# nullmax-vision/SimPB

Measured on AMD Instinct MI355X. Metric: frames/sec (6-cam sample) + MSDeformAttn HBM GB/s, R50 704x256 @1/2/4/8 GPU, higher is better.
Workload: dtype f32

## Files before the change

### include/simpb_hip.h

```cpp
#ifndef SIMPB_HIP_H
#define SIMPB_HIP_H

#ifdef __cplusplus
extern "C" {
#endif

#define SIMPB_OK 0
#define SIMPB_EINVAL 1
#define SIMPB_ELAUNCH 2

#define SIMPB_RECORD3D_WIDTH 15

int simpb_abi_version(void);

const char* simpb_last_error(void);

#define SIMPB_KERNEL_DAF 1
#define SIMPB_KERNEL_MSDA 2
int simpb_timing_enable(int capacity);
int simpb_timing_read(int kernel_id, float* ms_out, int max_n);
void simpb_timing_reset(void);

int simpb_deformable_aggregation_forward(
    float* output, const float* mc_ms_feat, const int* spatial_shape, const int* scale_start_index,
// ... 91 lines not shown
#define SIMPB_SURFACE_RGBA 13
int simpb_preprocess_planes_nhwc4_f16(void* out, const void* src, const void* image_table, void* mid, const int* kx,
                                      const int* xlo, const int* xn, const int* ky, const int* ylo, const int* yn,
                                      const void* lut, int num_images, int src_height, int src_width, int out_height,
                                      int out_width, int taps_x, int taps_y, int src_row0, int src_rows, int flip, int swap_rb,
                                      int format, long long pitch, long long chroma_pitch, long long chroma_offset,
                                      long long chroma2_offset, long long image_stride, int yoff, int iy, int irv, int igu,
                                      int igv, int ibu, void* stream);

int simpb_preprocess_mid_pitch(int out_width);

#define SIMPB_RIG_MAX_CAMS 16
typedef struct simpb_rig_camera {
  int format, src_height, src_width;
  int src_row0, src_rows, taps_x, taps_y, flip;
  long long pitch, chroma_pitch, chroma_offset;
  int kx_offset, x_offset, ky_offset, y_offset, mid_row;
  int yoff, iy, irv, igu, igv, ibu;
  long long chroma2_offset;
} simpb_rig_camera;
int simpb_preprocess_rig_nhwc4_f16(void* out, const void* image_table, void* mid, const int* kx, const int* xlo, const int* xn,
                                   const int* ky, const int* ylo, const int* yn, const void* lut, const simpb_rig_camera* cams,
                                   int num_cams, int num_images, int out_height, int out_width, int kx_len, int x_len, int ky_len,
                                   int y_len, int mid_rows, int swap_rb, void* stream);

#define SIMPB_PREPROCESS_MAX_ROLL_SIZE 8192
int simpb_preprocess_roll_nhwc4_f16(void* out, const void* src, const void* image_table, void* mid, const int* kx,
                                    const int* xlo, const int* xn, const int* ky, const int* ylo, const int* yn, const void* lut,
                                    int num_images, int src_height, int src_width, int out_height, int out_width, int taps_x,
                                    int taps_y, int src_row0, int src_rows, int flip, int swap_rb, int format, long long pitch,
                                    long long chroma_pitch, long long chroma_offset, long long chroma2_offset,
                                    long long image_stride, int yoff, int iy, int irv, int igu, int igv, int ibu, const int* roll,
                                    int roll_cams, void* stream);
int simpb_preprocess_rig_roll_nhwc4_f16(void* out, const void* image_table, void* mid, const int* kx, const int* xlo,
                                        const int* xn, const int* ky, const int* ylo, const int* yn, const void* lut,
                                        const simpb_rig_camera* cams, int num_cams, int num_images, int out_height, int out_width,
                                        int kx_len, int x_len, int ky_len, int y_len, int mid_rows, int swap_rb, const int* roll,
                                        void* stream);

#define SIMPB_GEMM_MAX_SEGS 4
#define SIMPB_GEMM_MAX_JOBS 4
#define SIMPB_GEMM_OUT_F32 0
#define SIMPB_GEMM_OUT_SPLIT_HALFS 1
typedef struct simpb_gemm_job {
  const float* x[SIMPB_GEMM_MAX_SEGS];
  int ldx[SIMPB_GEMM_MAX_SEGS];
  int kseg[SIMPB_GEMM_MAX_SEGS];
  int num_seg;
  int M, N, K;
  const float* w;
  const float* bias;
  float* y;
  const int* m_live;
  int ldw, ldy, relu;
  int out_fmt;
  const int* row_flag;
  const float* bias2;
  const void* w_hi;
  const void* w_lo;
} simpb_gemm_job;
typedef struct simpb_gemm_args {
  int num_jobs;
  int reserved;
  simpb_gemm_job job[SIMPB_GEMM_MAX_JOBS];
} simpb_gemm_args;
int simpb_gemm_f32(const simpb_gemm_args* args, void* stream);

int simpb_layernorm_f32(float* out, int ldo, const float* x0, int ld0, int k0, const float* x1, int ld1, int k1,
                        const float* gamma, const float* beta, int num_rows, const int* m_live, void* stream);

#define SIMPB_MAX_LEVELS 8
int simpb_format_tokens(float* col_feats, const void* const* level_ptrs, const void* const* level_bias,
                        const int* level_hw, int num_levels, int num_images, int channels, int src_is_half, void* stream);

int simpb_bias_act_nhwc_f16(void* y, const void* bias, const void* residual, long long num_pixels, int channels,
                            int relu, void* stream);

int simpb_bias_relu_maxpool_nhwc_f16(void* y, const void* x, const void* bias, int num_images, int in_h, int in_w,
                                     int channels, void* stream);

int simpb_conv1x1_nhwc_f16(void* y, const void* x, const void* weight, const void* bias, const void* residual,
                           int num_images, int in_h, int in_w, int in_channels, int out_channels, int stride, int relu,
                           int residual_upsample2x, const void* input_bias, int variant, void* stream);

int simpb_conv3x3_nhwc_f16(void* y, float* tokens, void* tokens_f16, int tokens_per_cam, int level_start, const void* x,
                           const void* weight, const void* bias, int num_images, int in_h, int in_w, int in_channels,
                           int out_channels, int stride, int relu, int variant, void* stream);

int simpb_conv3x3_choose_variant(long long p_out, int in_channels, int out_channels);

int simpb_conv3x3_choose_resident(long long p_out, int in_h, int in_w, int in_channels, int out_channels, int stride);

int simpb_conv3x3_group_choose_resident(int num_levels, int num_images, const int* in_h, const int* in_w, int in_channels,
                                        int out_channels);

int simpb_conv3x3_group_tokens_f16(int num_levels, float* tokens, void* tokens_f16, int tokens_per_cam, const int* level_start,
                                   const void* const* x, const void* const* weight, const void* const* bias, int num_images,
                                   const int* in_h, const int* in_w, int in_channels, int out_channels, int relu, void* stream);

int simpb_conv3x3_group_tokens_forms_f16(int num_levels, float* tokens, void* tokens_f16, int tokens_per_cam,
                                         const int* level_start, const void* const* x, const void* const* weight,
                                         const void* const* bias, int num_images, const int* in_h, const int* in_w,
                                         int in_channels, int out_channels, int relu, const int* variant, void* stream);

int simpb_stem_conv7x7_pool_f16_live(void* out, const void* img_nhwc4, const void* weight_packed, const void* bias,
                                     int num_images, int height, int width, int out_channels, void* stream, const int* live);
int simpb_conv1x1_nhwc_f16_live(void* y, const void* x, const void* weight, const void* bias, const void* residual,
                                int num_images, int in_h, int in_w, int in_channels, int out_channels, int stride, int relu,
                                int residual_upsample2x, const void* input_bias, int variant, void* stream, const int* live);
int simpb_conv3x3_nhwc_f16_live(void* y, float* tokens, void* tokens_f16, int tokens_per_cam, int level_start, const void* x,
                                const void* weight, const void* bias, int num_images, int in_h, int in_w, int in_channels,
                                int out_channels, int stride, int relu, int variant, void* stream, const int* live);
int simpb_conv3x3_group_tokens_forms_f16_live(int num_levels, float* tokens, void* tokens_f16, int tokens_per_cam,
                                              const int* level_start, const void* const* x, const void* const* weight,
                                              const void* const* bias, int num_images, const int* in_h, const int* in_w,
                                              int in_channels, int out_channels, int relu, const int* variant, void* stream,
                                              const int* live);

int simpb_attention_f32(float* out, const float* q, const float* k, const float* v, const int* query_cam,
                        const int* group_start, int batch_size, int num_heads, int head_dim, int num_query,
                        int num_key, int ldq, int ldk, int ldv, int ldo, float scale, void* stream);

int simpb_attention_f32_split(float* out, const float* q, const float* k, const float* v, const int* query_cam,
                              const int* group_start, int batch_size, int num_heads, int head_dim, int num_query,
                              int num_key, int ldq, int ldk, int ldv, int ldo, float scale, void* stream);

int simpb_attention_split_halfs(float* out, const void* q, const void* k, const void* v, const int* query_cam,
                                const int* group_start, int batch_size, int num_heads, int head_dim, int num_query,
                                int num_key, int ldq, int ldk, int ldv, int ldo, void* stream);

int simpb_attention_select(int split, float* out, const void* q, const void* k, const void* v, const void* k2, const void* v2,
                           const unsigned char* select, int batch_size, int num_heads, int head_dim, int num_query,
                           int num_key, int num_key2, int ldq, int ldk, int ldv, int ldk2, int ldv2, int ldo, float scale,
                           void* stream);

#define SIMPB_MLP_MAX_OPS 12
#define SIMPB_MLP_MAX_CHAINS 8
#define SIMPB_MLP_POST_NONE 0
#define SIMPB_MLP_POST_REFINE3D 1
#define SIMPB_MLP_POST_REFINE2D 2
#define SIMPB_MLP_POST_SIGMOID 3
#define SIMPB_MLP_LINEAR 0
#define SIMPB_MLP_LAYERNORM 1
#define SIMPB_MLP_IN_ROWS 0
#define SIMPB_MLP_IN_SINE2D 1
#define SIMPB_MLP_IN_ROWS_LN 2
typedef struct simpb_mlp_op {
  int type, in_dim, out_dim, relu;
  const float* w;
  const float* b;
} simpb_mlp_op;
typedef struct simpb_mlp_chain {
  const float* x;
  const float* x2;
  float* out;
  const float* out_scale;
  int ldx, ldx2, ldo, in_dim, in_mode, n_ops;
  int post, ldres, res_cols, div_rows, div_col0, reserved;
  const float* res;
  const float* div;
  simpb_mlp_op ops[SIMPB_MLP_MAX_OPS];
  const float* ln_w;
  const float* ln_b;
  float* ln_out;
  int ld_ln_out, reserved2;
} simpb_mlp_chain;
// ... 219 lines not shown
```

### simpb_amd/_lib.py

```python
import ctypes
import os

from .build import LIB

_lib = None

_P = ctypes.c_void_p
_I = ctypes.c_int
_F = ctypes.c_float
_LL = ctypes.c_longlong


class WorldTables(ctypes.Structure):
    _fields_ = [("class_range", _F * 32), ("attr_moving", ctypes.c_ubyte * 32), ("attr_still", ctypes.c_ubyte * 32),
                ("threshold", _F), ("has_threshold", _I), ("num_output", _I)]


class RigCamera(ctypes.Structure):
    _fields_ = ([(n, _I) for n in ("format", "src_height", "src_width", "src_row0", "src_rows", "taps_x", "taps_y", "flip")] +
                [(n, _LL) for n in ("pitch", "chroma_pitch", "chroma_offset")] +
                [(n, _I) for n in ("kx_offset", "x_offset", "ky_offset", "y_offset", "mid_row", "yoff", "iy", "irv", "igu", "igv", "ibu")] +
                [("chroma2_offset", _LL)])


class HealthParams(ctypes.Structure):
    _fields_ = [("dark_below", ctypes.c_double), ("bright_above", ctypes.c_double), ("flat_below", ctypes.c_double),
                ("mean", ctypes.c_double * 3), ("std", ctypes.c_double * 3),
                ("check_dark", _I), ("check_bright", _I), ("check_flat", _I), ("check_frozen", _I), ("frozen_after", _I), ("act", _I)]


SIGNATURES = {
    "simpb_abi_version": ([], _I),
    "simpb_last_error": ([], ctypes.c_char_p),
    "simpb_timing_enable": ([_I], _I),
    "simpb_timing_read": ([_I, _P, _I], _I),
    "simpb_timing_reset": ([], None),
    "simpb_deformable_aggregation_forward": ([_P] * 6 + [_I] * 8 + [_P], _I),
    "simpb_dfa_fused_forward": ([_P, _P, _I] + [_P] * 11 + [_I] * 9 + [_P], _I),
    "simpb_dfa_fused_forward_cams": ([_P, _P, _I] + [_P] * 11 + [_I] * 9 + [_P, _P], _I),
    "simpb_dfa_fused_forward_rig": ([_P, _P, _I] + [_P] * 11 + [_I] * 9 + [_P, _P], _I),
    "simpb_deformable_aggregation_backward": ([_P] * 9 + [_I] * 8 + [_P], _I),
    "simpb_ms_deform_attn_grouped_forward": ([_P] * 7 + [_I] * 8 + [_P], _I),
    "simpb_msda_linear_forward": ([_P, _I, _P, _I, _P, _P, _P, _I, _P, _I, _P, _P] + [_I] * 8 + [_P], _I),
    "simpb_ms_deform_attn_grouped_backward": ([_P] * 10 + [_I] * 8 + [_P], _I),
    "simpb_linear_f32": ([_P] * 4 + [_I] * 4 + [_P], _I),
    "simpb_linear_f16x3": ([_P] * 5 + [_I] * 3 + [_P], _I),
    "simpb_gemm_f32": ([_P, _P], _I),
    "simpb_layernorm_f32": ([_P, _I, _P, _I, _I, _P, _I, _I, _P, _P, _I, _P, _P], _I),
    "simpb_bias_act_nhwc_f16": ([_P, _P, _P, ctypes.c_longlong, _I, _I, _P], _I),
    "simpb_bias_relu_maxpool_nhwc_f16": ([_P, _P, _P, _I, _I, _I, _I, _P], _I),
    "simpb_conv1x1_nhwc_f16": ([_P] * 5 + [_I] * 8 + [_P, _I, _P], _I),
    "simpb_conv3x3_nhwc_f16": ([_P, _P, _P, _I, _I, _P, _P, _P] + [_I] * 8 + [_P], _I),
    "simpb_conv3x3_choose_variant": ([_LL, _I, _I], _I),
    "simpb_conv3x3_group_tokens_f16": ([_I, _P, _P, _I, _P, _P, _P, _P, _I, _P, _P, _I, _I, _I, _P], _I),
    "simpb_conv3x3_choose_resident": ([_LL, _I, _I, _I, _I, _I], _I),
    "simpb_conv3x3_group_choose_resident": ([_I, _I, _P, _P, _I, _I], _I),
    "simpb_conv3x3_group_tokens_forms_f16": ([_I, _P, _P, _I, _P, _P, _P, _P, _I, _P, _P, _I, _I, _I, _P, _P], _I),
    "simpb_stem_conv7x7_pool_f16": ([_P] * 4 + [_I] * 4 + [_P], _I),
    "simpb_stem_conv7x7_pool_f16_live": ([_P] * 4 + [_I] * 4 + [_P, _P], _I),
    "simpb_conv1x1_nhwc_f16_live": ([_P] * 5 + [_I] * 8 + [_P, _I, _P, _P], _I),
    "simpb_conv3x3_nhwc_f16_live": ([_P, _P, _P, _I, _I, _P, _P, _P] + [_I] * 8 + [_P, _P], _I),
    "simpb_conv3x3_group_tokens_forms_f16_live": ([_I, _P, _P, _I, _P, _P, _P, _P, _I, _P, _P, _I, _I, _I, _P, _P, _P], _I),
    "simpb_image_to_nhwc4_f16": ([_P, _P] + [ctypes.c_longlong] * 4 + [_I] * 4 + [_P], _I),
    "simpb_preprocess_u8_nhwc4_f16": ([_P] * 10 + [_I] * 11 + [_P], _I),
    "simpb_preprocess_yuv420sp_nhwc4_f16": ([_P] * 10 + [_I] * 18 + [_P], _I),
    "simpb_preprocess_surface_nhwc4_f16": ([_P] * 11 + [_I] * 12 + [_LL] * 4 + [_I] * 6 + [_P], _I),
    "simpb_preprocess_planes_nhwc4_f16": ([_P] * 11 + [_I] * 12 + [_LL] * 5 + [_I] * 6 + [_P], _I),
    "simpb_preprocess_mid_pitch": ([_I], _I),
    "simpb_preprocess_rig_nhwc4_f16": ([_P] * 10 + [ctypes.POINTER(RigCamera)] + [_I] * 10 + [_P], _I),
    "simpb_preprocess_roll_nhwc4_f16": ([_P] * 11 + [_I] * 12 + [_LL] * 5 + [_I] * 6 + [ctypes.POINTER(_I), _I, _P], _I),
    "simpb_preprocess_rig_roll_nhwc4_f16": ([_P] * 10 + [ctypes.POINTER(RigCamera)] + [_I] * 10 + [ctypes.POINTER(_I), _P], _I),
    "simpb_linear_f16in_split": ([_P] * 5 + [_I] * 3 + [_P], _I),
    "simpb_format_tokens": ([_P, _P, _P, _P, _I, _I, _I, _I, _P], _I),
    "simpb_attention_f32": ([_P] * 6 + [_I] * 9 + [_F, _P], _I),
    "simpb_attention_f32_split": ([_P] * 6 + [_I] * 9 + [_F, _P], _I),
    "simpb_attention_split_halfs": ([_P] * 6 + [_I] * 9 + [_P], _I),
    "simpb_attention_select": ([_I] + [_P] * 7 + [_I] * 12 + [_F, _P], _I),
    "simpb_mlp_chain_forward": ([_P, _P], _I),
    "simpb_bank_get": ([_P] * 6 + [_I] * 2 + [_F] * 2 + [_P], _I),
    "simpb_bank_get_restart": ([_P] * 6 + [_I] * 2 + [_F] * 2 + [_P, _P], _I),
    "simpb_bank_update": ([_P] * 10 + [_I] * 5 + [_P], _I),
    "simpb_bank_update_rank": ([_P, _P] + [_I] * 4 + [_P], _I),
    "simpb_bank_update_merge": ([_P] * 13 + [_I, _P] + [_I] * 5 + [_P], _I),
    "simpb_bank_update_merge_active": ([_P] * 13 + [_I, _P] + [_I] * 5 + [_P, _P], _I),
    "simpb_bank_cache": ([_P] * 10 + [_I] * 6 + [_F, _I, _F, _P, _I, _P, _P], _I),
    "simpb_bank_cache_streams": ([_P] * 10 + [_I] * 6 + [_F, _I, _F, _P, _I, _P, _P, _P], _I),
    "simpb_bank_cache_streams_active": ([_P] * 10 + [_I] * 6 + [_F, _I, _F, _P, _I, _P, _P, _P, _P], _I),
    "simpb_bank_cache_streams_restart": ([_P] * 10 + [_I] * 6 + [_F, _I, _F, _P, _I, _P, _P, _P, _P, _P], _I),
    "simpb_bank_export_stream": ([_P] * 5 + [_I] * 6 + [_P], _I),
    "simpb_bank_import_stream": ([_P] * 6 + [_I] * 6 + [_P], _I),
    "simpb_decode3d_record": ([_P] * 6 + [_I] * 4 + [_P], _I),
    "simpb_decode2d_record": ([_P] * 6 + [_I] * 4 + [_F] * 4 + [_P], _I),
    "simpb_record2d_compact": ([_P, _LL, _P, _LL, _I, _I, _I, _P], _I),
    "simpb_decode2d_record_ragged": ([_P] * 7 + [_I] * 5 + [_F] * 4 + [_P], _I),
    "simpb_decode2d_record_cams": ([_P] * 6 + [_I] * 4 + [_P, _I, _P], _I),
    "simpb_decode2d_record_ragged_cams": ([_P] * 7 + [_I] * 5 + [_P, _P], _I),
    "simpb_world_record": ([_P] * 5 + [WorldTables, _I, _P], _I),
    "simpb_image_health_stats": ([_P, _P, _I, _I, _I, _P], _I),
    "simpb_image_health_partials_bytes": ([_I, _I, _I], _I),
    "simpb_camera_health_verdict": ([_P] * 6 + [HealthParams] + [_I] * 4 + [_P], _I),
    "simpb_topk_rows": ([_P, _P, _P, _I, _I, _I, _P], _I),
    "simpb_rowdot_sigmoid": ([_P, _P, _I, _P, _P, _I, _I, _P, _P], _I),
    "simpb_anchor_projection": ([_P] * 4 + [_I] * 2 + [_P], _I),
    "simpb_msda_prep": ([_P, _P, _P, _I, _P, _I, _P, _I, _I, _I, _I, _P, _P], _I),
    "simpb_dfa_points": ([_P] * 7 + [_I] * 5 + [_P], _I),
    "simpb_dfa_weights": ([_P] * 3 + [_I] * 6 + [_P], _I),
    "simpb_dfa_points_cams": ([_P] * 7 + [_I] * 5 + [_P, _P], _I),
    "simpb_dfa_weights_cams": ([_P] * 3 + [_I] * 6 + [_P, _P], _I),
    "simpb_alloc_project_cams": ([_P] * 5 + [_I] * 3 + [_F] * 5 + [_P, _P], _I),
    "simpb_alloc_project": ([_P] * 5 + [_I] * 3 + [_F] * 5 + [_P], _I),
    "simpb_alloc_compact": ([_P] * 3 + [_I] * 3 + [_P], _I),
    "simpb_alloc_group_start": ([_P] * 3 + [_I] * 3 + [_P], _I),
    "simpb_alloc_scatter": ([_P] * 12 + [_I] * 4 + [_F] * 2 + [_P], _I),
    "simpb_alloc_static": ([_P] * 15 + [_I] * 4 + [_F] * 5 + [_P], _I),
    "simpb_alloc_ragged": ([_P] * 15 + [_I] * 4 + [_F] * 5 + [_P], _I),
    "simpb_alloc_ragged_active": ([_P] * 15 + [_I] * 4 + [_F] * 5 + [_P, _P], _I),
    "simpb_alloc_static_cams": ([_P] * 15 + [_I] * 4 + [_F] * 5 + [_P, _P], _I),
    "simpb_alloc_ragged_cams": ([_P] * 15 + [_I] * 4 + [_F] * 5 + [_P, _P, _P], _I),
    "simpb_gather_rows": ([_P] * 3 + [_I] * 4 + [_P], _I),
    "simpb_aggregate_2d_to_3d": ([_P] * 8 + [_I] * 5 + [_P], _I),
    "simpb_aggregate_2d_to_3d_alpha": ([_P] * 9 + [_I, _I, _P, _P] + [_I] * 5 + [_P], _I),
}

ERRORS = {1: "SIMPB_EINVAL (bad pointer/size/layout)", 2: "SIMPB_ELAUNCH (kernel launch failed)"}


def lib():
    global _lib
    if _lib is None:
        if not os.path.exists(LIB):
            raise RuntimeError(
                f"{LIB} is missing: build it with `python -m simpb_amd.build` (hipcc --offload-arch=gfx950). "
                "simpb_amd has no fallback path for its HIP kernels.")
        import torch
# ... 16 lines not shown
```

### simpb_amd/csrc/conv1x1.hip

```cpp
#include <hip/hip_runtime.h>
#include <hip/hip_fp16.h>
#include "../../include/simpb_hip.h"
#include "conv_parts.h"

#include "launch.h"
extern "C" int simpb_conv_pointwise_staged(void* y, const void* x, const void* weight, const void* bias, const void* residual,
                                           int p_out, int in_h, int in_w, int ho, int wo, int in_channels, int out_channels,
                                           int stride, int relu, int residual_upsample2x, int tiling, void* stream,
                                           const int* live);

namespace {

using namespace simpb::conv;

constexpr int BM = 128;

template <class... Lt>
__global__ __launch_bounds__(kThreads) void conv1x1_f16_kernel(_Float16* __restrict__ y, const _Float16* __restrict__ x,
                                                               const _Float16* __restrict__ w, const _Float16* __restrict__ bias,
                                                               const _Float16* __restrict__ residual, int P_out, int Cin,
                                                               int Cout, int relu, int stride, int Ho, int Wo, int H, int W,
                                                               int res_up, const _Float16* __restrict__ in_bias, const Lt... live) {
  constexpr bool LIVE = sizeof...(Lt) != 0;
  const LiveTable lt = table_of(live...);
// ... 35 lines not shown
  for (int i = 0; i < NB; ++i) brow[i] = (size_t)min(c0 + sr + RS * i, Cout - 1) * Cin + sc;
  const int nchunks = Cin / BK;
  h16x8 pa[2][NA], pb[2][NB], pin[2];
  auto fetch = [&](auto set_c, int chunk) __attribute__((always_inline)) {
    constexpr int set = decltype(set_c)::value;
    const int k0 = min(chunk, nchunks - 1) * BK;
    if (in_bias) pin[set] = *reinterpret_cast<const h16x8*>(in_bias + k0 + sc);
#pragma unroll
    for (int i = 0; i < NA; ++i) pa[set][i] = *reinterpret_cast<const h16x8*>(x + arow[i] + k0);
#pragma unroll
    for (int i = 0; i < NB; ++i) pb[set][i] = *reinterpret_cast<const h16x8*>(w + brow[i] + k0);
  };
  auto stash = [&](auto set_c, int) __attribute__((always_inline)) {
    constexpr int set = decltype(set_c)::value;
#pragma unroll
    for (int i = 0; i < NA; ++i) {
      h16x8 v = pa[set][i];
      if (in_bias) {
#pragma unroll
        for (int e = 0; e < 8; ++e) v[e] = (_Float16)fmaxf((float)v[e] + (float)pin[set][e], 0.f);
      }
      *reinterpret_cast<h16x8*>(&s_a[(sr + RS * i) * LDH + sc]) = v;
    }
#pragma unroll
    for (int i = 0; i < NB; ++i) *reinterpret_cast<h16x8*>(&s_b[(sr + RS * i) * LDH + sc]) = pb[set][i];
  };

  f32x16 acc[2];
  zero_acc(acc);

  auto multiply = [&]() __attribute__((always_inline)) {
#pragma unroll
    for (int ks = 0; ks < BK / 16; ++ks) {
      const h16x8 a = *reinterpret_cast<const h16x8*>(&s_a[(wave * 32 + r32) * LDH + 16 * ks + 8 * kb]);
#pragma unroll
      for (int n = 0; n < 2; ++n) {
        const h16x8 b = *reinterpret_cast<const h16x8*>(&s_b[(n * 32 + r32) * LDH + 16 * ks + 8 * kb]);
        acc[n] = simpb::mfma_32x32x16_f16(a, b, acc[n]);
      }
    }
  };

  const int pw = p0 + wave * 32;
  const int cl = c0 + (lane & 7) * 8;
  h16x8 rres[4] = {};
  if (residual && cl < Cout) {
#pragma unroll
    for (int i = 0; i < 4; ++i) {
      int p = real(min(pw + ((lane + 64 * i) >> 3), walked - 1));
      if (res_up) p = up2_row(p, Ho, Wo);
      rres[i] = *reinterpret_cast<const h16x8*>(residual + (size_t)p * Cout + cl);
    }
  }

  fetch(IC<0>{}, 0);
  fetch(IC<1>{}, 1);
  for (int c = 0; c < nchunks; c += 2) {
    __syncthreads();
    stash(IC<0>{}, c);
    __syncthreads();
    fetch(IC<0>{}, c + 2);
    multiply();
    if (c + 1 < nchunks) {
      __syncthreads();
      stash(IC<1>{}, c + 1);
      __syncthreads();
      fetch(IC<1>{}, c + 3);
      multiply();
    }
  }

  float* mine = s_c + wave * 32 * LDC;
  __syncthreads();
  acc_to_tile<2, LDC>(mine, acc, r32, kb);
  __syncthreads();
  if (cl >= Cout) return;
  const h16x8 bv = *reinterpret_cast<const h16x8*>(bias + cl);
  tile_pieces<2, LDC>(mine, 0, lane, [&](int i, int r, int, const float (&v)[8]) __attribute__((always_inline)) {
    const int p = LIVE ? real_row[wave * 32 + r] : pw + r;
    if (p < P_out) *reinterpret_cast<h16x8*>(y + (size_t)p * Cout + cl) = finish_piece(v, bv, rres[i], relu);
  });
}

}

extern "C" int simpb_conv1x1_nhwc_f16_live(void* y, const void* x, const void* weight, const void* bias, const void* residual,
                                           int num_images, int in_h, int in_w, int in_channels, int out_channels, int stride,
                                           int relu, int residual_upsample2x, const void* input_bias, int variant, void* stream,
                                           const int* live) {
  if (variant < 0 || variant > 4 || (input_bias && variant > 1)) return SIMPB_EINVAL;
  if (!y || !x || !weight || !bias || num_images <= 0 || in_h <= 0 || in_w <= 0 || in_channels <= 0 || out_channels <= 0 ||
      (stride != 1 && stride != 2) || in_channels % BK != 0 || out_channels % 8 != 0)
    return SIMPB_EINVAL;
  if ((reinterpret_cast<size_t>(y) | reinterpret_cast<size_t>(x) | reinterpret_cast<size_t>(weight) |
       reinterpret_cast<size_t>(bias) | reinterpret_cast<size_t>(residual) | reinterpret_cast<size_t>(input_bias)) & 15)
    return SIMPB_EINVAL;
  const int ho = (in_h - 1) / stride + 1, wo = (in_w - 1) / stride + 1;
  if (residual_upsample2x && (!residual || (ho & 1) || (wo & 1))) return SIMPB_EINVAL;
  const long long p_out = (long long)num_images * ho * wo;
  if (p_out > (1ll << 30)) return SIMPB_EINVAL;
  (void)hipGetLastError();
  if (variant == 0) {
    variant = (input_bias || in_channels < 512) ? 1 : 2;
    if (variant == 2 && in_channels >= 1024) {
      const long long t128 = ((p_out + 127) / 128) * ((out_channels + 63) / 64);
      if (t128 < 320) variant = 4;
    }
  }
  if (variant > 1) {
    if ((long long)num_images * in_h * in_w * in_channels > (1ll << 31) - 1) return SIMPB_EINVAL;
    return simpb_conv_pointwise_staged(y, x, weight, bias, residual, (int)p_out, in_h, in_w, ho, wo, in_channels, out_channels,
                                       stride, relu, residual_upsample2x, variant - 2, stream, live);
  }
  dim3 grid((unsigned)((p_out + BM - 1) / BM), (out_channels + BN - 1) / BN);
  if (grid.y > 65535) return SIMPB_EINVAL;
  if (!live)
    hipLaunchKernelGGL(conv1x1_f16_kernel<>, grid, dim3(kThreads), 0, static_cast<hipStream_t>(stream),
                       static_cast<_Float16*>(y), static_cast<const _Float16*>(x), static_cast<const _Float16*>(weight),
                       static_cast<const _Float16*>(bias), static_cast<const _Float16*>(residual), (int)p_out, in_channels,
                       out_channels, relu, stride, ho, wo, in_h, in_w, residual_upsample2x ? 1 : 0,
                       static_cast<const _Float16*>(input_bias));
  else
    hipLaunchKernelGGL(conv1x1_f16_kernel<LiveTable>, grid, dim3(kThreads), 0, static_cast<hipStream_t>(stream),
                       static_cast<_Float16*>(y), static_cast<const _Float16*>(x), static_cast<const _Float16*>(weight),
                       static_cast<const _Float16*>(bias), static_cast<const _Float16*>(residual), (int)p_out, in_channels, out_channels,
                       relu, stride, ho, wo, in_h, in_w, residual_upsample2x ? 1 : 0, static_cast<const _Float16*>(input_bias),
                       LiveTable{live, num_images});
  return simpb_check_launch();
}

extern "C" int simpb_conv1x1_nhwc_f16(void* y, const void* x, const void* weight, const void* bias, const void* residual,
                                      int num_images, int in_h, int in_w, int in_channels, int out_channels, int stride,
                                      int relu, int residual_upsample2x, const void* input_bias, int variant, void* stream) {
  return simpb_conv1x1_nhwc_f16_live(y, x, weight, bias, residual, num_images, in_h, in_w, in_channels, out_channels, stride, relu,
                                     residual_upsample2x, input_bias, variant, stream, nullptr);
}
```

### simpb_amd/plugin/ops.py

```python
import ctypes

import torch
from torch.autograd.function import Function

from .. import _lib


def _ptr(t):
    return ctypes.c_void_p(t.data_ptr())


def _stream():
    return ctypes.c_void_p(torch.cuda.current_stream().cuda_stream)


def _require_gpu(*tensors):
    for t in tensors:
        if not t.is_cuda:
            raise RuntimeError("simpb_amd operators run on the GPU only (got a CPU tensor); "
                               "there is no CPU fallback")


_layout_ok = {}

# ... 367 lines not shown
        raise ValueError("format_tokens takes f16/f32 levels with channels % 8 == 0")
    tokens = sum(h * w for h, w in shapes)
    col = torch.empty(bs, num_cams * tokens, c, device=levels[0].device, dtype=torch.float32)
    ptrs = (ctypes.c_void_p * len(srcs))(*[f.data_ptr() for f in srcs])
    hws = (ctypes.c_int * len(srcs))(*[h * w for h, w in shapes])
    bptrs = None
    if biases is not None:
        if len(biases) != len(srcs) or any(b is not None and (b.dtype != dtype or b.numel() != c or not b.is_contiguous()) for b in biases):
            raise ValueError("biases: one contiguous [C] tensor of the levels' dtype per level (or None)")
        bptrs = (ctypes.c_void_p * len(srcs))(*[b.data_ptr() if b is not None else None for b in biases])
    status = _lib.lib().simpb_format_tokens(_ptr(col), ptrs, bptrs, hws, len(srcs), bs * num_cams, c,
                                            1 if dtype == torch.float16 else 0, _stream())
    _lib.check(status, "simpb_format_tokens")
    spatial_shape, scale_start_index = _shape_tables(shapes, num_cams, col.device)
    return [col, spatial_shape, scale_start_index]


def bias_act_(y, bias, residual=None, relu=True):
    _require_gpu(y, bias)
    n, c, h, w = y.shape
    if (y.dtype != torch.float16 or not y.is_contiguous(memory_format=torch.channels_last) or bias.dtype != torch.float16
            or bias.numel() != c or c % 8):
        raise ValueError("bias_act_ takes a channels_last f16 tensor and an f16 bias with channels % 8 == 0")
    if residual is not None and (residual.shape != y.shape or residual.dtype != torch.float16
                                 or not residual.is_contiguous(memory_format=torch.channels_last)):
        raise ValueError("residual must match y (channels_last f16)")
    status = _lib.lib().simpb_bias_act_nhwc_f16(_ptr(y), _ptr(bias), _ptr(residual) if residual is not None else None,
                                                n * h * w, c, 1 if relu else 0, _stream())
    _lib.check(status, "simpb_bias_act_nhwc_f16")
    return y


def bias_relu_maxpool(x, bias):
    _require_gpu(x, bias)
    n, c, h, w = x.shape
    if (x.dtype != torch.float16 or not x.is_contiguous(memory_format=torch.channels_last) or bias.dtype != torch.float16
            or bias.numel() != c or c % 8 or not bias.is_contiguous()):
        raise ValueError("bias_relu_maxpool takes a channels_last f16 tensor and an f16 bias with channels % 8 == 0")
    y = torch.empty((n, c, (h - 1) // 2 + 1, (w - 1) // 2 + 1), device=x.device, dtype=torch.float16,
                    memory_format=torch.channels_last)
    _lib.check(_lib.lib().simpb_bias_relu_maxpool_nhwc_f16(_ptr(y), _ptr(x), _ptr(bias), n, h, w, c, _stream()),
               "simpb_bias_relu_maxpool_nhwc_f16")
    return y


def _live_ptr(live, n, device):
    if live is None:
        return None
    if live.dtype != torch.int32 or tuple(live.shape) != (1 + n,) or not live.is_contiguous() or live.device != device:
        raise ValueError(f"live: a contiguous i32 [{1 + n}] tensor on the images' device (runner.live_images)")
    return _ptr(live)


def conv1x1_nhwc(x, weight, bias, residual=None, relu=True, stride=1, residual_upsample2x=False, input_bias=None, variant=0,
                 live=None):
    _require_gpu(x, weight, bias)
    n, cin, h, w = x.shape
    cout = weight.shape[0]
    if (x.dtype != torch.float16 or not x.is_contiguous(memory_format=torch.channels_last) or weight.dtype != torch.float16
            or bias.dtype != torch.float16 or weight.numel() != cout * cin or cin % 64 or cout % 8 or stride not in (1, 2)):
        raise ValueError("conv1x1_nhwc takes channels_last f16 input, f16 [Cout, Cin, 1, 1] weight, Cin % 64 == 0, Cout % 8 == 0")
    ho, wo = (h - 1) // stride + 1, (w - 1) // stride + 1
    y = torch.empty((n, cout, ho, wo), device=x.device, dtype=torch.float16, memory_format=torch.channels_last)
    want = y.shape if not residual_upsample2x else (n, cout, ho // 2, wo // 2)
    if residual_upsample2x and (residual is None or ho % 2 or wo % 2):
        raise ValueError("residual_upsample2x needs a residual and even output sizes")
    if residual is not None and (tuple(residual.shape) != tuple(want) or residual.dtype != torch.float16
                                 or not residual.is_contiguous(memory_format=torch.channels_last)):
        raise ValueError("residual must match the output (channels_last f16)")
    if input_bias is not None and (input_bias.dtype != torch.float16 or input_bias.numel() != cin or not input_bias.is_contiguous()):
        raise ValueError("input_bias must be a contiguous f16 [Cin] tensor")
    w2 = weight.reshape(cout, cin)
    if not w2.is_contiguous():
        w2 = w2.contiguous()
    status = _lib.lib().simpb_conv1x1_nhwc_f16_live(_ptr(y), _ptr(x), _ptr(w2), _ptr(bias), _ptr(residual) if residual is not None else None,
                                                    n, h, w, cin, cout, stride, 1 if relu else 0,
                                                    1 if residual_upsample2x else 0,
                                                    _ptr(input_bias) if input_bias is not None else None, variant, _stream(),
                                                    _live_ptr(live, n, x.device))
    _lib.check(status, "simpb_conv1x1_nhwc_f16")
    return y


def conv3x3_nhwc(x, weight, bias, relu=True, stride=1, tokens=None, variant=0, live=None):
    _require_gpu(x, weight, bias)
    n, cin, h, w = x.shape
    cout = weight.shape[0]
    if (x.dtype != torch.float16 or not x.is_contiguous(memory_format=torch.channels_last) or weight.dtype != torch.float16
            or bias.dtype != torch.float16 or tuple(weight.shape) != (cout, cin, 3, 3) or cin % 64 or cout % 8
            or stride not in (1, 2) or bias.numel() != cout or not bias.is_contiguous()):
        raise ValueError("conv3x3_nhwc takes channels_last f16 input, f16 [Cout, Cin, 3, 3] weight, Cin % 64 == 0, Cout % 8 == 0")
    if not weight.is_contiguous(memory_format=torch.channels_last):
        weight = weight.contiguous(memory_format=torch.channels_last)
    ho, wo = (h - 1) // stride + 1, (w - 1) // stride + 1
    col16 = None
    if tokens is None:
        y = torch.empty((n, cout, ho, wo), device=x.device, dtype=torch.float16, memory_format=torch.channels_last)
        col, per_cam, start = None, 0, 0
    else:
        col, per_cam, start = tokens[:3]
        col16 = tokens[3] if len(tokens) > 3 else None
        y = None
        if col is None and col16 is None:
            raise ValueError("tokens: an f32 or an f16 token buffer")
        if col16 is not None and (col16.dtype != torch.float16 or not col16.is_contiguous()
                                  or (col is not None and col16.shape != col.shape)):
            raise ValueError("tokens: the f16 buffer must match col_feats")
        rows = col if col is not None else col16
        if ((col is not None and col.dtype != torch.float32) or not rows.is_contiguous() or rows.shape[-1] != cout
                or rows.numel() != n * per_cam * cout or start < 0 or start + ho * wo > per_cam):
            raise ValueError("tokens: (contiguous f32 [bs, cams * tokens_per_cam, Cout] with bs * cams == N, tokens_per_cam, level_start)")
    status = _lib.lib().simpb_conv3x3_nhwc_f16_live(_ptr(y) if y is not None else None, _ptr(col) if col is not None else None,
                                                    _ptr(col16) if col16 is not None else None, per_cam, start, _ptr(x), _ptr(weight), _ptr(bias), n, h, w, cin, cout, stride,
                                                    1 if relu else 0, variant, _stream(), _live_ptr(live, n, x.device))
    _lib.check(status, "simpb_conv3x3_nhwc_f16")
    return y


def conv3x3_variant_for(p_out, in_channels, out_channels):
    return int(_lib.lib().simpb_conv3x3_choose_variant(int(p_out), int(in_channels), int(out_channels)))


def conv3x3_resident_for(p_out, in_h, in_w, in_channels, out_channels, stride=1):
    return int(_lib.lib().simpb_conv3x3_choose_resident(int(p_out), int(in_h), int(in_w), int(in_channels), int(out_channels), int(stride)))


def conv3x3_group_resident_for(num_images, hws, in_channels, out_channels):
    import ctypes
    arr = ctypes.c_int * len(hws)
    return int(_lib.lib().simpb_conv3x3_group_choose_resident(len(hws), int(num_images), arr(*[int(h) for h, _ in hws]), arr(*[int(w) for _, w in hws]),
                                                              int(in_channels), int(out_channels)))


def conv3x3_group_tokens(xs, weights, biases, col, per_cam, starts, col16=None, relu=False, variants=None, live=None):
    import ctypes
    if col is None and col16 is None:
        raise ValueError("conv3x3_group_tokens: an f32 or an f16 token buffer")
    rows = col if col is not None else col16
    _require_gpu(*xs, *weights, *biases, rows)
    n, cin = xs[0].shape[:2]
    cout = weights[0].shape[0]
    k = len(xs)
    if not (1 <= k <= 4 and len(weights) == k and len(biases) == k and len(starts) == k):
        raise ValueError("conv3x3_group_tokens: 1..4 levels, one weight / bias / start each")
    ws = []
    for x, w, b in zip(xs, weights, biases):
        if (x.dtype != torch.float16 or not x.is_contiguous(memory_format=torch.channels_last) or x.shape[0] != n or x.shape[1] != cin
                or w.dtype != torch.float16 or tuple(w.shape) != (cout, cin, 3, 3) or b.dtype != torch.float16 or b.numel() != cout
                or not b.is_contiguous() or cin % 64 or cout % 8):
            raise ValueError("conv3x3_group_tokens takes channels_last f16 inputs of one channel count, f16 [Cout, Cin, 3, 3] weights")
        ws.append(w if w.is_contiguous(memory_format=torch.channels_last) else w.contiguous(memory_format=torch.channels_last))
    if ((col is not None and col.dtype != torch.float32) or not rows.is_contiguous() or rows.shape[-1] != cout
            or rows.numel() != n * per_cam * cout
            or (col16 is not None and (col16.dtype != torch.float16 or not col16.is_contiguous() or col16.shape != rows.shape))):
        raise ValueError("conv3x3_group_tokens: col = contiguous f32 [bs, cams * tokens_per_cam, Cout] with bs * cams == N")
    arr_p, arr_i = ctypes.c_void_p * k, ctypes.c_int * k
    if variants is not None and len(variants) != k:
        raise ValueError("conv3x3_group_tokens: one variant per level")
    status = _lib.lib().simpb_conv3x3_group_tokens_forms_f16_live(
        k, _ptr(col) if col is not None else None, _ptr(col16) if col16 is not None else None, int(per_cam), arr_i(*[int(v) for v in starts]),
        arr_p(*[x.data_ptr() for x in xs]), arr_p(*[w.data_ptr() for w in ws]), arr_p(*[b.data_ptr() for b in biases]), n,
        arr_i(*[x.shape[2] for x in xs]), arr_i(*[x.shape[3] for x in xs]), cin, cout, 1 if relu else 0,
        arr_i(*[int(v) for v in variants]) if variants is not None else None, _stream(), _live_ptr(live, n, xs[0].device))
    _lib.check(status, "simpb_conv3x3_group_tokens_forms_f16")


# ... 98 lines not shown
```

Before: 451.4.

## Add row-resident conv1x1 kernel that keeps input rows in LDS across output slabs

```diff
diff --git a/include/simpb_hip.h b/include/simpb_hip.h
--- a/include/simpb_hip.h
+++ b/include/simpb_hip.h
@@ -197,6 +197,8 @@
 int simpb_conv1x1_nhwc_f16(void* y, const void* x, const void* weight, const void* bias, const void* residual,
                            int num_images, int in_h, int in_w, int in_channels, int out_channels, int stride, int relu,
                            int residual_upsample2x, const void* input_bias, int variant, void* stream);
+
+int simpb_conv1x1_choose_variant(long long p_out, int in_channels, int out_channels, int stride, int has_input_bias);
 
 int simpb_conv3x3_nhwc_f16(void* y, float* tokens, void* tokens_f16, int tokens_per_cam, int level_start, const void* x,
                            const void* weight, const void* bias, int num_images, int in_h, int in_w, int in_channels,
diff --git a/simpb_amd/_lib.py b/simpb_amd/_lib.py
--- a/simpb_amd/_lib.py
+++ b/simpb_amd/_lib.py
@@ -50,6 +50,7 @@
     "simpb_bias_act_nhwc_f16": ([_P, _P, _P, ctypes.c_longlong, _I, _I, _P], _I),
     "simpb_bias_relu_maxpool_nhwc_f16": ([_P, _P, _P, _I, _I, _I, _I, _P], _I),
     "simpb_conv1x1_nhwc_f16": ([_P] * 5 + [_I] * 8 + [_P, _I, _P], _I),
+    "simpb_conv1x1_choose_variant": ([_LL, _I, _I, _I, _I], _I),
     "simpb_conv3x3_nhwc_f16": ([_P, _P, _P, _I, _I, _P, _P, _P] + [_I] * 8 + [_P], _I),
     "simpb_conv3x3_choose_variant": ([_LL, _I, _I], _I),
     "simpb_conv3x3_group_tokens_f16": ([_I, _P, _P, _I, _P, _P, _P, _P, _I, _P, _P, _I, _I, _I, _P], _I),
diff --git a/simpb_amd/csrc/conv1x1.hip b/simpb_amd/csrc/conv1x1.hip
--- a/simpb_amd/csrc/conv1x1.hip
+++ b/simpb_amd/csrc/conv1x1.hip
@@ -141,13 +141,236 @@
   });
 }
 
+constexpr int LDT = 33;
+
+template <int BMr, int CIN>
+constexpr size_t rows_lds() {
+  return (size_t)BMr * (CIN + 8) * 2 + 2 * BN * LDH * 2 + 4 * 32 * LDT * 4;
+}
+
+__device__ __forceinline__ void wave_tile_sync() {
+  __builtin_amdgcn_fence(__ATOMIC_RELEASE, "wavefront");
+  __builtin_amdgcn_wave_barrier();
+  __builtin_amdgcn_fence(__ATOMIC_ACQUIRE, "wavefront");
+}
+
+template <int BMr, int CIN, class... Lt>
+__global__ __launch_bounds__(kThreads) void conv1x1_rows_kernel(_Float16* __restrict__ y, const _Float16* __restrict__ x,
+                                                                const _Float16* __restrict__ w, const _Float16* __restrict__ bias,
+                                                                const _Float16* __restrict__ residual, int P_out, int Cout,
+                                                                int slab, int relu, int stride, int Ho, int Wo, int H, int W,
+                                                                int res_up, const _Float16* __restrict__ in_bias, const Lt... live) {
+  constexpr bool LIVE = sizeof...(Lt) != 0;
+  constexpr int WM = BMr / 32, WN = 4 / WM, NF = 2 / WN;
+  constexpr int LDX = CIN + 8, KT = CIN / BK;
+  static_assert((BMr == 64 || BMr == 128) && CIN % BK == 0 && (CIN / 8) % 2 == 0 && kThreads % (CIN / 8) == 0, "tile");
+  const LiveTable lt = table_of(live...);
+  const int walked = LIVE ? live_count(lt) * Ho * Wo : P_out;
+  const int p0 = blockIdx.x * BMr;
+  if constexpr (LIVE) {
+    if (p0 >= walked) return;
+  }
+  auto real = [&](int p) __attribute__((always_inline)) {
+    if constexpr (LIVE) return live_pixel(lt, p, Ho * Wo);
+    else return p;
+  };
+  extern __shared__ __attribute__((aligned(16))) unsigned char rows_smem[];
+  _Float16* s_x = reinterpret_cast<_Float16*>(rows_smem);
+  _Float16* s_w = s_x + BMr * LDX;
+  float* s_t = reinterpret_cast<float*>(s_w + 2 * BN * LDH);
+  const int tid = threadIdx.x;
+  const int lane = tid & 63, wave = tid >> 6;
+  const int r32 = lane & 31, kb = lane >> 5;
+  const int wm = wave % WM, wn = wave / WM;
+  const int s0 = blockIdx.y * slab;
+  const int nsteps = (min(slab, Cout - s0) + BN - 1) / BN, T = nsteps * KT;
+  float* mine = s_t + wave * 32 * LDT;
+
+  const int c8 = (lane & 3) * 8;
+  size_t rsrc[2];
+  long long ydst[2];
+#pragma unroll
+  for (int ps = 0; ps < 2; ++ps) {
+    const int prow = p0 + wm * 32 + (lane >> 2) + 16 * ps;
+    int p = real(min(prow, walked - 1));
+    ydst[ps] = prow < walked ? (long long)p * Cout : -1;
+    if (res_up) p = up2_row(p, Ho, Wo);
+    rsrc[ps] = (size_t)p * Cout;
+  }
+  auto frag_channel = [&](int step, int f) __attribute__((always_inline)) { return s0 + step * BN + (WN == 2 ? wn : f) * 32 + c8; };
+  auto fetch_step = [&](h16x8 (&rr)[NF][2], h16x8 (&bb)[NF], int step) __attribute__((always_inline)) {
+#pragma unroll
+    for (int f = 0; f < NF; ++f) {
+      const int cl = frag_channel(step, f);
+      const bool in = step < nsteps && cl < Cout;
+      bb[f] = h16x8{};
+      if (in) bb[f] = *reinterpret_cast<const h16x8*>(bias + cl);
+#pragma unroll
+      for (int ps = 0; ps < 2; ++ps) {
+        rr[f][ps] = h16x8{};
+        if (in && residual) rr[f][ps] = *reinterpret_cast<const h16x8*>(residual + rsrc[ps] + cl);
+      }
+    }
+  };
+  h16x8 rcur[NF][2], rnext[NF][2], bcur[NF], bnext[NF];
+  fetch_step(rcur, bcur, 0);
+
+  const int wr = tid >> 3, wc = (tid & 7) * 8;
+  h16x8 pw[2][2];
+  auto fetch_w = [&](auto set_c, int t) __attribute__((always_inline)) {
+    constexpr int set = decltype(set_c)::value;
+    const int tc = min(t, T - 1), step = tc / KT, k0 = (tc - step * KT) * BK;
+#pragma unroll
+    for (int i = 0; i < 2; ++i)
+      pw[set][i] = *reinterpret_cast<const h16x8*>(w + (size_t)min(s0 + step * BN + wr + 32 * i, Cout - 1) * CIN + k0 + wc);
+  };
+  auto stash_w = [&](auto set_c, int buf) __attribute__((always_inline)) {
+    constexpr int set = decltype(set_c)::value;
+#pragma unroll
+    for (int i = 0; i < 2; ++i) *reinterpret_cast<h16x8*>(&s_w[(buf * BN + wr + 32 * i) * LDH + wc]) = pw[set][i];
+  };
+  fetch_w(IC<0>{}, 0);
+  fetch_w(IC<1>{}, 1);
+
+  {
+    constexpr int PRX = CIN / 8, XRS = kThreads / PRX, NX = BMr / XRS, XB = NX < 8 ? NX : 8;
+    const int xr = tid / PRX, xc = (tid % PRX) * 8;
+    h16x8 pin = {};
+    if (in_bias) pin = *reinterpret_cast<const h16x8*>(in_bias + xc);
+#pragma unroll
+    for (int i0 = 0; i0 < NX; i0 += XB) {
+      h16x8 px[XB];
+#pragma unroll
+      for (int i = 0; i < XB; ++i) {
+        int p = real(min(p0 + xr + XRS * (i0 + i), walked - 1));
+        if (stride != 1) {
+          const Pixel q = split_pixel(p, Ho, Wo);
+          p = (q.n * H + q.ho * stride) * W + q.wo * stride;
+        }
+        px[i] = *reinterpret_cast<const h16x8*>(x + (size_t)p * CIN + xc);
+      }
+#pragma unroll
+      for (int i = 0; i < XB; ++i) {
+        h16x8 v = px[i];
+        if (in_bias) {
+#pragma unroll
+          for (int e = 0; e < 8; ++e) v[e] = (_Float16)fmaxf((float)v[e] + (float)pin[e], 0.f);
+        }
+        *reinterpret_cast<h16x8*>(&s_x[(xr + XRS * (i0 + i)) * LDX + xc]) = v;
+      }
+    }
+  }
+  stash_w(IC<0>{}, 0);
+  fetch_w(IC<0>{}, 2);
+  __syncthreads();
+
+  f32x16 acc[NF][1];
+  zero_acc(acc);
+
+  auto tile = [&](auto set_c, int t) __attribute__((always_inline)) {
+    constexpr int S = decltype(set_c)::value;
+    const int step = t / KT, chunk = t - step * KT;
+    if (t + 1 < T) {
+      stash_w(IC<S ^ 1>{}, S ^ 1);
+      fetch_w(IC<S ^ 1>{}, t + 3);
+    }
+    if (chunk == 0) fetch_step(rnext, bnext, step + 1);
+    __builtin_amdgcn_sched_barrier(0);
+#pragma unroll
+    for (int ks = 0; ks < BK / 16; ++ks) {
+      const h16x8 a = *reinterpret_cast<const h16x8*>(&s_x[(wm * 32 + r32) * LDX + chunk * BK + 16 * ks + 8 * kb]);
+#pragma unroll
+      for (int f = 0; f < NF; ++f) {
+        const h16x8 b = *reinterpret_cast<const h16x8*>(&s_w[(S * BN + (WN == 2 ? wn : f) * 32 + r32) * LDH + 16 * ks + 8 * kb]);
+        acc[f][0] = simpb::mfma_32x32x16_f16(a, b, acc[f][0]);
+      }
+    }
+    if (chunk == KT - 1) {
+#pragma unroll
+      for (int f = 0; f < NF; ++f) {
+        const int cl = frag_channel(step, f);
+        acc_to_tile<1, LDT>(mine, acc[f], r32, kb);
+        wave_tile_sync();
+        tile_pieces<1, LDT>(mine, 0, lane, [&](int ps, int, int, const float (&v)[8]) __attribute__((always_inline)) {
+          if (ydst[ps] >= 0 && cl < Cout)
+            *reinterpret_cast<h16x8*>(y + ydst[ps] + cl) = finish_piece(v, bcur[f], rcur[f][ps], relu);
+        });
+        wave_tile_sync();
+      }
+      zero_acc(acc);
+#pragma unroll
+      for (int f = 0; f < NF; ++f) {
+        bcur[f] = bnext[f];
+#pragma unroll
+        for (int ps = 0; ps < 2; ++ps) rcur[f][ps] = rnext[f][ps];
+      }
+    }
+    __syncthreads();
+  };
+  for (int t = 0; t < T; t += 2) {
+    tile(IC<0>{}, t);
+    if (t + 1 < T) tile(IC<1>{}, t + 1);
+  }
+}
+
+struct RowsForm {
+  int bm, slab;
+};
+inline RowsForm rows_form(int in_channels, int out_channels) {
+  if (out_channels <= BN) return {0, 0};
+  if (in_channels == 64) return {64, out_channels};
+  if (in_channels == 128) return {64, out_channels < 256 ? out_channels : 256};
+  return {0, 0};
+}
+
+template <int BMr, int CIN>
+int launch_rows(const RowsForm& f, void* y, const void* x, const void* weight, const void* bias, const void* residual, long long p_out,
+                int out_channels, int relu, int stride, int ho, int wo, int in_h, int in_w, int res_up, const void* input_bias,
+                hipStream_t stream, const int* live, int num_images) {
+  constexpr size_t lds = rows_lds<BMr, CIN>();
+  const dim3 grid((unsigned)((p_out + BMr - 1) / BMr), (unsigned)((out_channels + f.slab - 1) / f.slab));
+  if (grid.y > 65535) return SIMPB_EINVAL;
+  if (!live) {
+    static const bool allowed = hipFuncSetAttribute(reinterpret_cast<const void*>(conv1x1_rows_kernel<BMr, CIN>),
+                                                    hipFuncAttributeMaxDynamicSharedMemorySize, (int)lds) == hipSuccess;
+    (void)allowed;
+    hipLaunchKernelGGL((conv1x1_rows_kernel<BMr, CIN>), grid, dim3(kThreads), lds, stream, static_cast<_Float16*>(y),
+                       static_cast<const _Float16*>(x), static_cast<const _Float16*>(weight), static_cast<const _Float16*>(bias),
+                       static_cast<const _Float16*>(residual), (int)p_out, out_channels, f.slab, relu, stride, ho, wo, in_h, in_w,
+                       res_up, static_cast<const _Float16*>(input_bias));
+  } else {
+    static const bool allowed = hipFuncSetAttribute(reinterpret_cast<const void*>(conv1x1_rows_kernel<BMr, CIN, LiveTable>),
+                                                    hipFuncAttributeMaxDynamicSharedMemorySize, (int)lds) == hipSuccess;
+    (void)allowed;
+    hipLaunchKernelGGL((conv1x1_rows_kernel<BMr, CIN, LiveTable>), grid, dim3(kThreads), lds, stream, static_cast<_Float16*>(y),
+                       static_cast<const _Float16*>(x), static_cast<const _Float16*>(weight), static_cast<const _Float16*>(bias),
+                       static_cast<const _Float16*>(residual), (int)p_out, out_channels, f.slab, relu, stride, ho, wo, in_h, in_w,
+                       res_up, static_cast<const _Float16*>(input_bias), LiveTable{live, num_images});
+  }
+  return simpb_check_launch();
+}
+
+}
+
+extern "C" int simpb_conv1x1_choose_variant(long long p_out, int in_channels, int out_channels, int stride, int has_input_bias) {
+  if (stride == 1 && in_channels == 64 && out_channels == 256 && p_out >= 65536) return 5;
+  if (stride == 1 && in_channels == 128 && out_channels == 512 && p_out >= 16384) return 5;
+  if (!has_input_bias && in_channels == 256 &&
+      ((stride == 1 && out_channels <= 256 && p_out >= 65536) || (stride == 2 && out_channels == 512 && p_out >= 16384)))
+    return 4;
+  int variant = (has_input_bias || in_channels < 512) ? 1 : 2;
+  if (variant == 2 && in_channels >= 1024) {
+    const long long t128 = ((p_out + 127) / 128) * ((out_channels + 63) / 64);
+    if (t128 < 320) variant = 4;
+  }
+  return variant;
 }
 
 extern "C" int simpb_conv1x1_nhwc_f16_live(void* y, const void* x, const void* weight, const void* bias, const void* residual,
                                            int num_images, int in_h, int in_w, int in_channels, int out_channels, int stride,
                                            int relu, int residual_upsample2x, const void* input_bias, int variant, void* stream,
                                            const int* live) {
-  if (variant < 0 || variant > 4 || (input_bias && variant > 1)) return SIMPB_EINVAL;
+  if (variant < 0 || variant > 5 || (input_bias && variant > 1 && variant < 5)) return SIMPB_EINVAL;
   if (!y || !x || !weight || !bias || num_images <= 0 || in_h <= 0 || in_w <= 0 || in_channels <= 0 || out_channels <= 0 ||
       (stride != 1 && stride != 2) || in_channels % BK != 0 || out_channels % 8 != 0)
     return SIMPB_EINVAL;
@@ -159,12 +382,16 @@
   const long long p_out = (long long)num_images * ho * wo;
   if (p_out > (1ll << 30)) return SIMPB_EINVAL;
   (void)hipGetLastError();
-  if (variant == 0) {
-    variant = (input_bias || in_channels < 512) ? 1 : 2;
-    if (variant == 2 && in_channels >= 1024) {
-      const long long t128 = ((p_out + 127) / 128) * ((out_channels + 63) / 64);
-      if (t128 < 320) variant = 4;
-    }
+  if (variant == 0) variant = simpb_conv1x1_choose_variant(p_out, in_channels, out_channels, stride, input_bias ? 1 : 0);
+  if (variant == 5) {
+    const RowsForm f = rows_form(in_channels, out_channels);
+    if (!f.bm) return SIMPB_EINVAL;
+    auto go = [&](auto cin_c) {
+      return launch_rows<64, decltype(cin_c)::value>(f, y, x, weight, bias, residual, p_out, out_channels, relu, stride, ho, wo, in_h, in_w,
+                                                     residual_upsample2x ? 1 : 0, input_bias, static_cast<hipStream_t>(stream), live,
+                                                     num_images);
+    };
+    return in_channels == 64 ? go(IC<64>{}) : go(IC<128>{});
   }
   if (variant > 1) {
     if ((long long)num_images * in_h * in_w * in_channels > (1ll << 31) - 1) return SIMPB_EINVAL;
diff --git a/simpb_amd/plugin/ops.py b/simpb_amd/plugin/ops.py
--- a/simpb_amd/plugin/ops.py
+++ b/simpb_amd/plugin/ops.py
@@ -473,6 +473,11 @@
     return y
 
 
+def conv1x1_variant_for(p_out, in_channels, out_channels, stride=1, input_bias=False):
+    return int(_lib.lib().simpb_conv1x1_choose_variant(int(p_out), int(in_channels), int(out_channels), int(stride),
+                                                       1 if input_bias else 0))
+
+
 def conv3x3_nhwc(x, weight, bias, relu=True, stride=1, tokens=None, variant=0, live=None):
     _require_gpu(x, weight, bias)
     n, cin, h, w = x.shape
```

After: 454.7 (median of 5 runs). About the same (+0.7%).
